# thu-ml/SageAttention

Hardware: AMD Instinct MI355X
Metric: attention TFLOPS (causal, hd=128), kernel-only, as published by the reference (higher is better)
Workload: dtype int8 QK^T + fp8(e4m3) PV, fp32 accumulate

## Files before the change

sageattention_amd/csrc/sage_prepass.hip:

```cpp
#include "sage_common.h"
#include "sage_kernels.h"
#include "sage_quant_math.h"
#include <type_traits>

#ifndef SAGE_PP_RELEASE
#define SAGE_PP_RELEASE 0
#endif
#ifndef SAGE_PP_NT
#define SAGE_PP_NT 1
#endif
#ifndef SAGE_PP_TRACE
#define SAGE_PP_TRACE 0
#endif
#ifndef SAGE_PP_KWB
#define SAGE_PP_KWB 1
#endif
#ifndef SAGE_PP_VAMAX
#define SAGE_PP_VAMAX 1
#endif
#ifndef SAGE_PP_ABL
#define SAGE_PP_ABL 0
#endif

namespace sage {

template <int DT> __device__ __forceinline__ void round_pair_to_dtype(float &a, float &b)
{
    if constexpr (DT == DT_BF16) {
        typedef float f2 __attribute__((ext_vector_type(2)));
        typedef __bf16 b2 __attribute__((ext_vector_type(2)));
        const b2 r = __builtin_convertvector(f2{a, b}, b2);
        unsigned u;
        __builtin_memcpy(&u, &r, 4);
        a = __uint_as_float(u << 16);
        b = __uint_as_float(u & 0xffff0000u);
    } else {
        a = f16_to_f32(f32_to_f16_rne(a));
        b = f16_to_f32(f32_to_f16_rne(b));
    }
}

constexpr int kPrepassThreads = 512;

template <int DT> __device__ __forceinline__ unsigned pack_pair_to_dtype(float a, float b)
{
    typedef float f2 __attribute__((ext_vector_type(2)));
    unsigned u;
    if constexpr (DT == DT_BF16) {
        typedef __bf16 b2 __attribute__((ext_vector_type(2)));
        const b2 r = __builtin_convertvector(f2{a, b}, b2);
        __builtin_memcpy(&u, &r, 4);
    } else {
        typedef _Float16 h2 __attribute__((ext_vector_type(2)));
        const h2 r = __builtin_convertvector(f2{a, b}, h2);
        __builtin_memcpy(&u, &r, 4);
    }
    return u;
}

template <int D>
struct PrepassLds {
    static constexpr int TPR = D / 4, RPI = kPrepassThreads / TPR, LDT = D + 8;
    float red[3][RPI][D];
    __attribute__((aligned(16))) uint16_t tile[2][BLKK * LDT];
    float ch_mean[D], ch_recp[D];
    uint16_t kmean[D];
    unsigned failed;
    unsigned gmax[8][8];
    float gsc[8][8], gy[8][8];
};

template <int D, int DT, bool IS_V, bool VARLEN, bool V_AMAX = false>
__device__ __forceinline__ void prepass_body(const PrepassParams &p, PrepassLds<D> &lds, const int b)
{

    constexpr int NT = kPrepassThreads;
    constexpr int TPR = D / 4;
    constexpr int RPI = NT / TPR;
    constexpr int NR = kStatsSlab / RPI;
    constexpr int LDT = D + 8;
    auto &red = lds.red; auto &tile = lds.tile; auto &ch_mean = lds.ch_mean; auto &ch_recp = lds.ch_recp;
    auto &kmean = lds.kmean; auto &gmax = lds.gmax; auto &gsc = lds.gsc; auto &gy = lds.gy;
    bool failed = false;
    constexpr int is_v = IS_V ? 1 : 0;

    const int tid = threadIdx.x;
    const int gslab = blockIdx.x, h = blockIdx.y;
    int slab = gslab, L = p.L, nslab = p.nslab;
    long tok0 = 0, tile0 = 0;
    bool gap = false;
    if constexpr (VARLEN) {
        typedef const __attribute__((address_space(4))) int *cint_p;
        nslab = ((cint_p)p.hdr)[4];
        if (gslab >= nslab) return;
        const int seg = ((cint_p)p.slab_seq)[gslab];
        slab = gslab - ((cint_p)p.slab_first)[seg];
        int t0, len;
        varlen_segment((cint_p)p.cu, p.nseq, p.L, seg, t0, len);
        tok0 = t0;
        L = len;
        gap = seg >= p.nseq;
        if (gap && (IS_V || p.k_mean == nullptr)) return;
        tile0 = gap ? 0 : ((cint_p)p.cu_tiles)[seg];
    }
    const long bh = (long)b * p.H + h;
    const long x_sl = is_v ? p.v_sl : p.k_sl;
    const uint16_t *x = (is_v ? reinterpret_cast<const uint16_t *>(p.v) + (long)b * p.v_sb + (long)h * p.v_sh
                              : reinterpret_cast<const uint16_t *>(p.k) + (long)b * p.k_sb + (long)h * p.k_sh) + tok0 * x_sl;
    const int c4 = (tid % TPR) * 4, r0 = tid / TPR;
    const int row0 = slab * kStatsSlab;
    const int end = min(L, row0 + kStatsSlab);
    const int my_rows = (end - row0 - r0 + RPI - 1) / RPI;
#if SAGE_PP_TRACE
    unsigned long long *trace = reinterpret_cast<unsigned long long *>(p.ws + 2L * p.B * p.H * p.nslab * 3 * D) +
                                8L * (blockIdx.x + gridDim.x * (blockIdx.y + (long)gridDim.y * blockIdx.z));
    int tslot = 0;
#define SAGE_STAMP() do { if (tid == 0) trace[tslot] = wall_clock64(); tslot++; } while (0)
    SAGE_STAMP();
#else
#define SAGE_STAMP() do { } while (0)
#endif

    unsigned rw[NR][2];
    {
        const unsigned head_bytes = (unsigned)(((long)(L - 1) * x_sl + D) * 2);
        const __amdgpu_buffer_rsrc_t rsrc = __builtin_amdgcn_make_buffer_rsrc(const_cast<uint16_t *>(x), 0, head_bytes, 0x00020000);
        const unsigned toff = (unsigned)((row0 + r0) * (int)x_sl + c4) * 2u;
        const unsigned step = (unsigned)(RPI * (int)x_sl) * 2u;
        unsigned voff = toff;
#pragma unroll
        for (int i = 0; i < NR; i++) {
            const v2u t = __builtin_amdgcn_raw_buffer_load_b64(rsrc, voff, 0, 0);
            rw[i][0] = t[0]; rw[i][1] = t[1];
            voff += step;
            asm volatile("" : "+v"(voff));
        }
    }
#if SAGE_PP_TRACE
    { unsigned acc = 0;
#pragma unroll
      for (int i = 0; i < NR; i++) acc += rw[i][0] ^ rw[i][1];
      if (acc == 0x12345u) p.ws[0] = 1.0f; }
    SAGE_STAMP();
#endif

    const bool need_stats = IS_V ? (p.v_fp16 == 0) : (p.k_mean != nullptr);
    if (need_stats) {
        float mx[4], mn[4], sm[4];
#pragma unroll
        for (int j = 0; j < 4; j++) { mx[j] = -INFINITY; mn[j] = INFINITY; sm[j] = 0.0f; }
        if constexpr (V_AMAX) {
            typedef unsigned short us2 __attribute__((ext_vector_type(2)));
            us2 am01 = {0, 0}, am23 = {0, 0};
#pragma unroll
            for (int i = 0; i < ((SAGE_PP_ABL & 4) ? 0 : NR); i++) {
                const unsigned m0 = rw[i][0] & 0x7fff7fffu, m1 = rw[i][1] & 0x7fff7fffu;
                us2 a, b;
                __builtin_memcpy(&a, &m0, 4);
                __builtin_memcpy(&b, &m1, 4);
                am01 = __builtin_elementwise_max(am01, a);
                am23 = __builtin_elementwise_max(am23, b);
                asm volatile("" : "+v"(am01), "+v"(am23) :: "memory");
            }
            mx[0] = ld16<DT>(am01[0]); mx[1] = ld16<DT>(am01[1]); mx[2] = ld16<DT>(am23[0]); mx[3] = ld16<DT>(am23[1]);
#pragma unroll
            for (int j = 0; j < 4; j++) mn[j] = 0.0f;
        } else if (!(SAGE_PP_ABL & 4)) {
#pragma unroll
            for (int i = 0; i < NR; i++) {
                float pen = 0.0f;
                if constexpr (IS_V) pen = __uint_as_float((unsigned)((my_rows - 1 - i) >> 31) & 0xff800000u);
#pragma unroll
                for (int c = 0; c < 2; c++) {
                    const unsigned w = rw[i][c];
                    const float lo = ld16<DT>((uint16_t)(w & 0xffffu)), hi = ld16<DT>((uint16_t)(w >> 16));
                    if constexpr (IS_V) {
                        mx[2 * c] = fmaxf(mx[2 * c], lo + pen);         mn[2 * c] = fminf(mn[2 * c], lo - pen);
                        mx[2 * c + 1] = fmaxf(mx[2 * c + 1], hi + pen); mn[2 * c + 1] = fminf(mn[2 * c + 1], hi - pen);
                    }
                    sm[2 * c] += lo;
                    sm[2 * c + 1] += hi;
                }
                asm volatile("" : "+v"(sm[0]), "+v"(sm[1]), "+v"(sm[2]), "+v"(sm[3]) :: "memory");
            }
        }
#pragma unroll
        for (int j = 0; j < 4; j++) { red[0][r0][c4 + j] = mx[j]; red[1][r0][c4 + j] = mn[j]; red[2][r0][c4 + j] = sm[j]; }
        __syncthreads();
        float *ws = p.ws + (((long)is_v * p.B * p.H + bh) * p.nslab) * 3 * D;
        if (tid < D) {
            float a = -INFINITY, c = INFINITY, s = 0.0f;
#pragma unroll
            for (int r = 0; r < RPI; r++) { a = fmaxf(a, red[0][r][tid]); c = fminf(c, red[1][r][tid]); s += red[2][r][tid]; }
            float *mine = ws + (long)gslab * 3 * D;
            if constexpr (IS_V) __hip_atomic_store(mine + tid, a, __ATOMIC_RELAXED, __HIP_MEMORY_SCOPE_AGENT);
            if constexpr (IS_V && !V_AMAX) __hip_atomic_store(mine + D + tid, c, __ATOMIC_RELAXED, __HIP_MEMORY_SCOPE_AGENT);
            if constexpr (!V_AMAX) __hip_atomic_store(mine + 2 * D + tid, s, __ATOMIC_RELAXED, __HIP_MEMORY_SCOPE_AGENT);
        }
        SAGE_STAMP();
        unsigned *cnt = p.sync + ((long)is_v * p.B * p.H + bh) * kPrepassSyncStride;
        if (nslab > 1 && !(SAGE_PP_ABL & 1)) {
            asm volatile("s_waitcnt vmcnt(0)" ::: "memory");
            __syncthreads();
            if (tid == 0) {
                __hip_atomic_fetch_add(cnt, 1u, SAGE_PP_RELEASE ? __ATOMIC_RELEASE : __ATOMIC_RELAXED, __HIP_MEMORY_SCOPE_AGENT);
                const unsigned want = (unsigned)nslab + (p.debug_fail ? 1u : 0u);
                const long long bound = p.debug_fail ? 20000LL : 3000000LL;
                const unsigned min_polls = p.debug_fail ? (1u << 8) : (1u << 14);
                const long long t0 = wall_clock64();
                unsigned gave_up = 0, polls = 0;
                while (__hip_atomic_load(cnt, __ATOMIC_RELAXED, __HIP_MEMORY_SCOPE_AGENT) < want) {
                    __builtin_amdgcn_s_sleep(2);
                    if (++polls > min_polls && wall_clock64() - t0 > bound) {
                        __hip_atomic_store(cnt + 2, 1u, __ATOMIC_RELAXED, __HIP_MEMORY_SCOPE_AGENT);
                        if (p.host_flag != nullptr) __hip_atomic_store(p.host_flag, 1u, __ATOMIC_RELAXED, __HIP_MEMORY_SCOPE_SYSTEM);
                        gave_up = 1;
                        break;
                    }
                }
                lds.failed = gave_up;
            }
            __syncthreads();
            failed = lds.failed != 0;
        }
        SAGE_STAMP();
        float a = -INFINITY, c = INFINITY, s = 0.0f;
        if (failed) {
            for (int i = 0; i < nslab; i++) {
                const uint16_t *xi = x;
                int Li = L, si = i;
                if constexpr (VARLEN) {
                    typedef const __attribute__((address_space(4))) int *cint_p;
                    const int seg = ((cint_p)p.slab_seq)[i];
                    si = i - ((cint_p)p.slab_first)[seg];
                    int t0;
                    varlen_segment((cint_p)p.cu, p.nseq, p.L, seg, t0, Li);
                    xi = x + ((long)t0 - tok0) * x_sl;
                }
                const int rbeg = si * kStatsSlab + r0, rend = min(Li, si * kStatsSlab + kStatsSlab);
                float fx[4], fn[4], fs[4];
#pragma unroll
                for (int j = 0; j < 4; j++) { fx[j] = V_AMAX ? 0.0f : -INFINITY; fn[j] = V_AMAX ? 0.0f : INFINITY; fs[j] = 0.0f; }
                const __amdgpu_buffer_rsrc_t rs_i = __builtin_amdgcn_make_buffer_rsrc(const_cast<uint16_t *>(xi), 0,
                                                                                      (unsigned)(((long)(Li - 1) * x_sl + D) * 2), 0x00020000);
                unsigned vo = (unsigned)(rbeg * (int)x_sl + c4) * 2u;
#pragma nounroll
                for (int r = rbeg; r < rend; r += RPI) {
                    const v2u t = __builtin_amdgcn_raw_buffer_load_b64(rs_i, vo, 0, 0);
                    vo += (unsigned)(RPI * (int)x_sl) * 2u;
#pragma unroll
                    for (int j = 0; j < 4; j++) {
                        const unsigned w = t[j >> 1];
                        const float f = ld16<DT>((uint16_t)((j & 1) ? (w >> 16) : (w & 0xffffu)));
                        if constexpr (V_AMAX) fx[j] = fmaxf(fx[j], fabsf(f));
                        else if constexpr (IS_V) { fx[j] = fmaxf(fx[j], f); fn[j] = fminf(fn[j], f); fs[j] += f; }
                        else fs[j] += f;
                    }
                }
                __syncthreads();
#pragma unroll
                for (int j = 0; j < 4; j++) {
                    if constexpr (IS_V) red[0][r0][c4 + j] = fx[j];
                    if constexpr (IS_V && !V_AMAX) red[1][r0][c4 + j] = fn[j];
                    if constexpr (!V_AMAX) red[2][r0][c4 + j] = fs[j];
                }
                __syncthreads();
                if (tid < D) {
                    float ai = -INFINITY, ci = INFINITY, s_i = 0.0f;
#pragma unroll
                    for (int r = 0; r < RPI; r++) {
                        if constexpr (IS_V) ai = fmaxf(ai, red[0][r][tid]);
                        if constexpr (IS_V && !V_AMAX) ci = fminf(ci, red[1][r][tid]);
                        if constexpr (!V_AMAX) s_i += red[2][r][tid];
                    }
                    if constexpr (IS_V) a = fmaxf(a, ai);
                    if constexpr (IS_V && !V_AMAX) c = fminf(c, ci);
                    if constexpr (!V_AMAX) s += s_i;
                }
            }
        } else if (tid < D) {
            constexpr int NB = (D == 128) ? 16 : 8;
            for (int i0 = 0; i0 < nslab; i0 += NB) {
                float va[NB], vc[NB], vs[NB];
#pragma unroll
                for (int u = 0; u < NB; u++) {
                    const float *wi = ws + (long)min(i0 + u, nslab - 1) * 3 * D;
                    if constexpr (IS_V) va[u] = __hip_atomic_load(wi + tid, __ATOMIC_RELAXED, __HIP_MEMORY_SCOPE_AGENT);
                    if constexpr (IS_V && !V_AMAX) vc[u] = __hip_atomic_load(wi + D + tid, __ATOMIC_RELAXED, __HIP_MEMORY_SCOPE_AGENT);
                    if constexpr (!V_AMAX) vs[u] = __hip_atomic_load(wi + 2 * D + tid, __ATOMIC_RELAXED, __HIP_MEMORY_SCOPE_AGENT);
                }
#pragma unroll
                for (int u = 0; u < NB; u++) {
                    if (i0 + u < nslab) {
                        if constexpr (IS_V) a = fmaxf(a, va[u]);
                        if constexpr (IS_V && !V_AMAX) c = fminf(c, vc[u]);
                        if constexpr (!V_AMAX) s += vs[u];
                    }
                }
            }
        }
        if (tid < D) {
            if constexpr (!IS_V) {
                const uint16_t m = st16<DT>(s / (float)(VARLEN ? p.L : L));
                kmean[tid] = m;
                if (gslab == 0) reinterpret_cast<uint16_t *>(p.k_mean)[bh * D + tid] = m;
            } else {
                const bool smooth = p.v_mean != nullptr;
                const float lpad = (float)((L + 15) / 16 * 16);
                const float mean = smooth ? s / lpad : 0.0f;
                if constexpr (V_AMAX) c = 0.0f;
                if ((L & 15) != 0) { a = fmaxf(a, 0.0f); c = fminf(c, 0.0f); }
                const float am = fmaxf(fabsf(a - mean), fabsf(c - mean));
                ch_mean[tid] = mean;
                ch_recp[tid] = am > 0.0f ? p.scale_max / am : 0.0f;
                if (gslab == 0) {
                    p.v_scale[bh * D + tid] = am / p.scale_max;
                    if (smooth) p.v_mean[bh * D + tid] = mean;
                }
            }
        }
        __syncthreads();
        SAGE_STAMP();
        if (nslab > 1 && tid == 0 && !(SAGE_PP_ABL & 1)) {
            const unsigned left = __hip_atomic_fetch_add(cnt + 1, 1u, __ATOMIC_RELAXED, __HIP_MEMORY_SCOPE_AGENT);
            if (left == (unsigned)nslab - 1) {
                __hip_atomic_store(cnt, 0u, __ATOMIC_RELAXED, __HIP_MEMORY_SCOPE_AGENT);
                __hip_atomic_store(cnt + 1, 0u, __ATOMIC_RELAXED, __HIP_MEMORY_SCOPE_AGENT);
            }
        }
    }
    if (gap) return;
    if (SAGE_PP_ABL & 2) {
        unsigned acc = 0;
#pragma unroll
        for (int i = 0; i < NR; i++) acc += rw[i][0] + rw[i][1];
        if (acc == 0x12345u) p.ws[0] = 1.0f;
        return;
    }

    if constexpr (!IS_V) {
        const int blk = p.k_blk;
        const int bsh = (blk == 128) ? 7 : 6;
        const int nb = kStatsSlab >> bsh;
        const int ngroups = (p.k_gran == GR_BLOCK) ? 1 : 4 * (blk / p.k_warp);
        const bool smooth = p.k_mean != nullptr;
        const unsigned init_bits = (p.k_style == QS_CUDA) ? __float_as_uint(1e-7f) : 0u;
        if (tid < 64) gmax[tid >> 3][tid & 7] = init_bits;
        float mean4[4] = {0.0f, 0.0f, 0.0f, 0.0f};
        unsigned m01 = 0u, m23 = 0u;
        if (smooth) {
            m01 = (unsigned)kmean[c4] | ((unsigned)kmean[c4 + 1] << 16);
            m23 = (unsigned)kmean[c4 + 2] | ((unsigned)kmean[c4 + 3] << 16);
#pragma unroll
            for (int j = 0; j < 4; j++) mean4[j] = ld16<DT>(kmean[c4 + j]);
        }
#pragma unroll
        for (int i = 0; i < NR; i++) {
            const unsigned gone = (unsigned)((my_rows - 1 - i) >> 31);
            rw[i][0] |= m01 & gone;
            rw[i][1] |= m23 & gone;
        }
#if SAGE_PP_KWB
        if (smooth && p.k_style != QS_CUDA) {
#pragma unroll
            for (int i = 0; i < NR; i++) {
#pragma unroll
                for (int c = 0; c < 2; c++) {
                    unsigned u = rw[i][c];
                    const float lo = ld16<DT>((uint16_t)(u & 0xffffu)) - mean4[2 * c];
                    const float hi = ld16<DT>((uint16_t)(u >> 16)) - mean4[2 * c + 1];
                    u = pack_pair_to_dtype<DT>(lo, hi);
                    asm volatile("" : "+v"(u));
                    rw[i][c] = u;
                }
                asm volatile("" ::: "memory");
            }
        }
#endif
        __syncthreads();
        const int g_thread = group_of_row(r0 & (blk - 1), p.k_gran, p.k_warp);
        const int nblk_total = (L + blk - 1) >> bsh;
        const __amdgpu_buffer_rsrc_t orsrc = __builtin_amdgcn_make_buffer_rsrc(
            p.k_out + (long)b * p.ko_sb + (long)h * p.ko_sh + tok0 * p.ko_sl, 0, (unsigned)((long)(L - 1) * p.ko_sl + D), 0x00020000);
        const unsigned ooff = (unsigned)((row0 + r0) * (int)p.ko_sl + c4), ostep = (unsigned)(RPI * (int)p.ko_sl);

        auto quantise = [&](auto style_tag, auto smooth_tag) {
            constexpr int STYLE = decltype(style_tag)::value;
            constexpr bool SMOOTH = decltype(smooth_tag)::value;
            auto row_values = [&](int i, float (&f)[4]) {
#pragma unroll
                for (int c = 0; c < 2; c++) {
                    unsigned w = rw[i][c];
                    asm volatile("" : "+v"(w));
                    float lo = ld16<DT>((uint16_t)(w & 0xffffu)), hi = ld16<DT>((uint16_t)(w >> 16));
                    if constexpr (SMOOTH) {
                        lo -= mean4[2 * c];
                        hi -= mean4[2 * c + 1];
                        if (STYLE != 0) round_pair_to_dtype<DT>(lo, hi);
                    }
                    f[2 * c] = lo;
                    f[2 * c + 1] = hi;
                }
            };
            const int rb_mask = (blk / RPI) - 1;
            float amax = 0.0f;
            typedef unsigned short us2 __attribute__((ext_vector_type(2)));
            us2 amax16 = {0, 0};
#pragma unroll
            for (int i = 0; i < NR; i++) {
                if constexpr (STYLE == 0) {
                    float f[4];
                    row_values(i, f);
                    amax = fmaxf(fmaxf(amax, fmaxf(fabsf(f[0]), fabsf(f[1]))), fmaxf(fabsf(f[2]), fabsf(f[3])));
                } else {
#pragma unroll
                    for (int c = 0; c < 2; c++) {
                        unsigned u = rw[i][c];
                        if constexpr (SMOOTH) {
                            asm volatile("" : "+v"(u));
                            const float lo = ld16<DT>((uint16_t)(u & 0xffffu)) - mean4[2 * c];
                            const float hi = ld16<DT>((uint16_t)(u >> 16)) - mean4[2 * c + 1];
                            u = pack_pair_to_dtype<DT>(lo, hi);
                        }
                        const unsigned mag = u & 0x7fff7fffu;
                        us2 m2;
                        __builtin_memcpy(&m2, &mag, 4);
                        amax16 = __builtin_elementwise_max(amax16, m2);
                    }
                }
                if ((i & 1) && ((i & rb_mask) == rb_mask)) {
                    float m = amax;
                    if constexpr (STYLE != 0) { m = ld16<DT>(amax16[0] > amax16[1] ? amax16[0] : amax16[1]); amax16 = us2{0, 0}; }
                    m = fmaxf(m, __uint_as_float(__builtin_amdgcn_update_dpp(0, __float_as_uint(m), 0xB1, 0xf, 0xf, true)));
                    m = fmaxf(m, __uint_as_float(__builtin_amdgcn_update_dpp(0, __float_as_uint(m), 0x4E, 0xf, 0xf, true)));
                    m = fmaxf(m, __uint_as_float(__builtin_amdgcn_update_dpp(0, __float_as_uint(m), 0x141, 0xf, 0xf, true)));
                    m = fmaxf(m, __uint_as_float(__builtin_amdgcn_update_dpp(0, __float_as_uint(m), 0x140, 0xf, 0xf, true)));
                    m = fmaxf(m, __shfl_xor(m, 16));
                    if ((tid & 31) == 0) atomicMax(&gmax[(i * RPI) >> bsh][g_thread], __float_as_uint(m));
                    amax = 0.0f;
                }
                asm volatile("" : "+v"(amax), "+v"(amax16) :: "memory");
            }
            __syncthreads();
            SAGE_STAMP();
            if (tid < nb * ngroups) {
                const int kb = tid / ngroups, g = tid % ngroups;
                const int gb = slab * nb + kb;
                const float am = __uint_as_float(gmax[kb][g]);
                const float sc = quant_scale(am, p.k_style);
                gsc[kb][g] = sc;
                gy[kb][g] = (STYLE == 0) ? 127.0f / am : quant_recip(sc);
                float *ksc_out = VARLEN ? p.k_scale + (tile0 + gb) * p.H + h
                                        : p.k_scale + (bh * nblk_total + gb) * ngroups + g;
                if (gb < nblk_total) *ksc_out = sc;
            }
            __syncthreads();
            unsigned orun = ooff;
#pragma unroll
            for (int i = 0; i < NR; i += 2) {
                const float sc = gsc[(i * RPI) >> bsh][g_thread], y = gy[(i * RPI) >> bsh][g_thread];
#pragma unroll
                for (int u = 0; u < 2; u++) {
                    float f[4];
                    row_values(i + u, f);
                    int q[4];
                    if constexpr (STYLE == 0) {
#pragma unroll
                        for (int j = 0; j < 4; j++) q[j] = quant_round_cuda(f[j], y);
                    } else if constexpr (STYLE == 1) quant_round_triton_nz4(f, sc, y, q);
                    else quant_round_triton4(f, sc, y, q);
                    __builtin_amdgcn_raw_buffer_store_b32(pack_int8x4(q[0], q[1], q[2], q[3]), orsrc, orun, 0, SAGE_PP_NT ? 2 : 0);
                    orun += ostep;
                    asm volatile("" : "+v"(orun) :: "memory");
                }
            }
        };
        auto by_smooth = [&](auto style_tag) {
            if (smooth) quantise(style_tag, std::true_type{}); else quantise(style_tag, std::false_type{});
        };
        if (p.k_style == QS_CUDA) by_smooth(std::integral_constant<int, 0>{});
#if SAGE_PP_KWB
        else if (p.k_style == QS_TRITON_THREAD) quantise(std::integral_constant<int, 1>{}, std::false_type{});
        else quantise(std::integral_constant<int, 2>{}, std::false_type{});
#else
        else if (p.k_style == QS_TRITON_THREAD) by_smooth(std::integral_constant<int, 1>{});
        else by_smooth(std::integral_constant<int, 2>{});
#endif
    } else {
        const bool smooth = V_AMAX ? false : (p.v_mean != nullptr);
        const int ntiles = (L + BLKK - 1) / BLKK;
        constexpr int RPS = 2 * BLKK / RPI;
        auto stage_in = [&](int s) {
#pragma unroll
            for (int m = 0; m < RPS; m++) {
                const int rs = r0 + m * RPI;
                const v2u t = {rw[s * RPS + m][0], rw[s * RPS + m][1]};
                *reinterpret_cast<v2u *>(&tile[rs >> 6][(rs & 63) * LDT + c4]) = t;
            }
        };
        if (p.v_fp16 == 0) {
            unsigned char *img = reinterpret_cast<unsigned char *>(p.v_image) + bh * (long)ntiles * (D * 64);
#pragma unroll
            for (int s = 0; s < kStatsSlab / (2 * BLKK); s++) {
                if (row0 + s * 2 * BLKK < L) {
                    stage_in(s);
                    __syncthreads();
#pragma unroll
                    for (int it = 0; it < 2 * D * 4 / NT; it++) {
                        const int piece = tid + NT * it;
                        const int tt = piece / (D * 4), pin = piece % (D * 4);
                        const int d = pin >> 2, pc = pin & 3;
                        const int t = (row0 >> 6) + 2 * s + tt;
                        if (t >= ntiles) continue;
                        const int ch = swz_chunk<64>(d, pc);
                        const float mean = ch_mean[d], recp = ch_recp[d];
                        float f[16];
#pragma unroll
                        for (int j = 0; j < 16; j++) {
                            const int tok = pv_token_of_position(16 * ch + j);
                            float xv = ld16<DT>(tile[tt][tok * LDT + d]);
                            if (smooth) xv = (t * BLKK + tok < L) ? xv - mean : 0.0f;
                            xv *= recp;
                            f[j] = fminf(fmaxf(xv, -448.0f), 448.0f);
                        }
                        v4u pk;
#pragma unroll
                        for (int w = 0; w < 4; w++) {
                            int word = __builtin_amdgcn_cvt_pk_fp8_f32(f[4 * w], f[4 * w + 1], 0, false);
                            word = __builtin_amdgcn_cvt_pk_fp8_f32(f[4 * w + 2], f[4 * w + 3], word, true);
                            pk[w] = (unsigned)word;
                        }
                        if constexpr (SAGE_PP_NT != 0) __builtin_nontemporal_store(pk, reinterpret_cast<v4u *>(img + (long)t * (D * 64) + d * 64 + pc * 16));
                        else *reinterpret_cast<v4u *>(img + (long)t * (D * 64) + d * 64 + pc * 16) = pk;
                    }
                    __syncthreads();
                }
            }
        } else {
            const long img_t = VARLEN ? (long)p.H * (D * 128) : (long)(D * 128);
            unsigned char *img = reinterpret_cast<unsigned char *>(p.v_image) + (VARLEN ? (tile0 * p.H + h) * (long)(D * 128) : bh * (long)ntiles * (D * 128));
#pragma unroll
            for (int s = 0; s < kStatsSlab / (2 * BLKK); s++) {
                if (row0 + s * 2 * BLKK < L) {
                    stage_in(s);
                    __syncthreads();
#pragma unroll
                    for (int it = 0; it < 2 * D * 8 / NT; it++) {
                        const int piece = tid + NT * it;
                        const int tt = piece / (D * 8), pin = piece % (D * 8);
                        const int d = pin >> 3, pc = pin & 7;
                        const int t = (row0 >> 6) + 2 * s + tt;
                        if (t >= ntiles) continue;
                        const int ch = swz_chunk<128>(d, pc);
                        v4u pk;
#pragma unroll
                        for (int w = 0; w < 4; w++) {
                            unsigned word = 0;
#pragma unroll
                            for (int e = 0; e < 2; e++) {
                                const int tok = pv_token_of_position(8 * ch + 2 * w + e);
                                uint16_t raw = tile[tt][tok * LDT + d];
                                if (DT != DT_F16) raw = f32_to_f16_rne(bf16_to_f32(raw));
                                word |= (unsigned)raw << (16 * e);
                            }
                            pk[w] = word;
                        }
                        if constexpr (SAGE_PP_NT != 0) __builtin_nontemporal_store(pk, reinterpret_cast<v4u *>(img + (long)t * img_t + d * 128 + pc * 16));
                        else *reinterpret_cast<v4u *>(img + (long)t * img_t + d * 128 + pc * 16) = pk;
                    }
                    __syncthreads();
                }
            }
        }
    }
#if SAGE_PP_TRACE
    asm volatile("s_waitcnt vmcnt(0)" ::: "memory");
    if (is_v) tslot = 6;
    SAGE_STAMP();
    if (tid == 0) trace[7] = (unsigned long long)__builtin_amdgcn_s_getreg((3 << 11) | 20) |
                              ((unsigned long long)__builtin_amdgcn_s_getreg((31 << 11) | 4) << 8);
#endif
}

template <int D, int DT, bool VARLEN>
#ifndef SAGE_PP_WAVES
#define SAGE_PP_WAVES 4
#endif
#ifndef SAGE_PP_WAVES64
#define SAGE_PP_WAVES64 6
#endif
__global__ void __launch_bounds__(kPrepassThreads, (D == 64 ? SAGE_PP_WAVES64 : SAGE_PP_WAVES))
prepass_kv_kernel(const PrepassParams p)
{
    __shared__ PrepassLds<D> lds;
    const int is_v = (p.parts == 3) ? (int)(blockIdx.z & 1) : (p.parts == 2);
    const int b = (p.parts == 3) ? (int)(blockIdx.z >> 1) : (int)blockIdx.z;
    if (is_v) {
        if (SAGE_PP_VAMAX && !VARLEN && p.v_mean == nullptr && p.v_fp16 == 0) prepass_body<D, DT, true, VARLEN, true>(p, lds, b);
        else prepass_body<D, DT, true, VARLEN>(p, lds, b);
    } else prepass_body<D, DT, false, VARLEN>(p, lds, b);
}

__global__ void __launch_bounds__(1024) debug_spin_kernel(long long ticks)
{
    const long long t0 = wall_clock64();
    while (wall_clock64() - t0 < ticks) __builtin_amdgcn_s_sleep(8);
}

hipError_t launch_debug_spin(int ms, int nwg, hipStream_t s)
{
    hipLaunchKernelGGL(debug_spin_kernel, dim3(nwg), dim3(1024), 0, s, (long long)ms * 100000LL);
    return hipGetLastError();
}

hipError_t launch_prepass_kv(const PrepassParams &p, hipStream_t s)
{
    if (p.B <= 0 || p.H <= 0 || p.nslab <= 0 || p.parts == 0) return hipSuccess;
    dim3 grid(p.nslab, p.H, p.B * (p.parts == 3 ? 2 : 1));
#define SAGE_PP(D_, T_) do { if (p.cu != nullptr) hipLaunchKernelGGL((prepass_kv_kernel<D_, T_, true>), grid, dim3(kPrepassThreads), 0, s, p); \
                             else hipLaunchKernelGGL((prepass_kv_kernel<D_, T_, false>), grid, dim3(kPrepassThreads), 0, s, p); } while (0)
    if (p.D == 128) { if (p.dtype == DT_F16) SAGE_PP(128, DT_F16); else SAGE_PP(128, DT_BF16); }
    else if (p.D == 64) { if (p.dtype == DT_F16) SAGE_PP(64, DT_F16); else SAGE_PP(64, DT_BF16); }
    else return hipErrorInvalidValue;
#undef SAGE_PP
    return hipGetLastError();
}

}
```

Before: 1612.

## Use swizzled LDS units with transpose reads and double-buffering in V prepass

Replaces the padded LDS tile in the V prepass with XOR-swizzled unit buffers (one aliased with the reduction scratch) that are read back through ds_read_tr16 transpose loads. Each lane now gathers four tokens per instruction instead of scalar 16-bit loads. Staging of the next unit is overlapped with converting the current one, which removes one barrier per step. It also drops unused stats reductions, skips the K padding fix-up when the slab is full, moves the gmax init earlier to remove a barrier, and swaps a shuffle for permlane16_swap. In exchange the swizzle and lane-mapping logic is intricate and relies on gfx950-only instructions.

```diff
diff --git a/sageattention_amd/csrc/sage_prepass.hip b/sageattention_amd/csrc/sage_prepass.hip
--- a/sageattention_amd/csrc/sage_prepass.hip
+++ b/sageattention_amd/csrc/sage_prepass.hip
@@ -60,9 +60,18 @@
 
 template <int D>
 struct PrepassLds {
-    static constexpr int TPR = D / 4, RPI = kPrepassThreads / TPR, LDT = D + 8;
-    float red[3][RPI][D];
-    __attribute__((aligned(16))) uint16_t tile[2][BLKK * LDT];
+    static constexpr int TPR = D / 4, RPI = kPrepassThreads / TPR;
+    static constexpr int UT = BLKK * 8 / (D / 16), UNIT = UT * D;
+    union {
+        __attribute__((aligned(16))) float red[3][RPI][D];
+        __attribute__((aligned(16))) uint16_t unit1[UNIT];
+    };
+    __attribute__((aligned(16))) uint16_t unit0[UNIT];
+    static __device__ __forceinline__ int tile_off(int row, int chunk, int col)
+    {
+        const int swz = (D == 128) ? ((row & 7) ^ ((row >> 2) & 4)) : (((row >> 1) & 3) ^ ((row >> 3) & 2));
+        return row * D + 16 * (chunk ^ swz) + col;
+    }
     float ch_mean[D], ch_recp[D];
     uint16_t kmean[D];
     unsigned failed;
@@ -78,8 +87,7 @@
     constexpr int TPR = D / 4;
     constexpr int RPI = NT / TPR;
     constexpr int NR = kStatsSlab / RPI;
-    constexpr int LDT = D + 8;
-    auto &red = lds.red; auto &tile = lds.tile; auto &ch_mean = lds.ch_mean; auto &ch_recp = lds.ch_recp;
+    auto &red = lds.red; auto &ch_mean = lds.ch_mean; auto &ch_recp = lds.ch_recp;
     auto &kmean = lds.kmean; auto &gmax = lds.gmax; auto &gsc = lds.gsc; auto &gy = lds.gy;
     bool failed = false;
     constexpr int is_v = IS_V ? 1 : 0;
@@ -145,6 +153,10 @@
 #endif
 
     const bool need_stats = IS_V ? (p.v_fp16 == 0) : (p.k_mean != nullptr);
+    if constexpr (!IS_V) {
+        const unsigned init_bits = (p.k_style == QS_CUDA) ? __float_as_uint(1e-7f) : 0u;
+        if (tid < 64) gmax[tid >> 3][tid & 7] = init_bits;
+    }
     if (need_stats) {
         float mx[4], mn[4], sm[4];
 #pragma unroll
@@ -185,13 +197,21 @@
             }
         }
 #pragma unroll
-        for (int j = 0; j < 4; j++) { red[0][r0][c4 + j] = mx[j]; red[1][r0][c4 + j] = mn[j]; red[2][r0][c4 + j] = sm[j]; }
+        for (int j = 0; j < 4; j++) {
+            if constexpr (IS_V) red[0][r0][c4 + j] = mx[j];
+            if constexpr (IS_V && !V_AMAX) red[1][r0][c4 + j] = mn[j];
+            if constexpr (!V_AMAX) red[2][r0][c4 + j] = sm[j];
+        }
         __syncthreads();
         float *ws = p.ws + (((long)is_v * p.B * p.H + bh) * p.nslab) * 3 * D;
         if (tid < D) {
             float a = -INFINITY, c = INFINITY, s = 0.0f;
 #pragma unroll
-            for (int r = 0; r < RPI; r++) { a = fmaxf(a, red[0][r][tid]); c = fminf(c, red[1][r][tid]); s += red[2][r][tid]; }
+            for (int r = 0; r < RPI; r++) {
+                if constexpr (IS_V) a = fmaxf(a, red[0][r][tid]);
+                if constexpr (IS_V && !V_AMAX) c = fminf(c, red[1][r][tid]);
+                if constexpr (!V_AMAX) s += red[2][r][tid];
+            }
             float *mine = ws + (long)gslab * 3 * D;
             if constexpr (IS_V) __hip_atomic_store(mine + tid, a, __ATOMIC_RELAXED, __HIP_MEMORY_SCOPE_AGENT);
             if constexpr (IS_V && !V_AMAX) __hip_atomic_store(mine + D + tid, c, __ATOMIC_RELAXED, __HIP_MEMORY_SCOPE_AGENT);
@@ -344,8 +364,6 @@
         const int nb = kStatsSlab >> bsh;
         const int ngroups = (p.k_gran == GR_BLOCK) ? 1 : 4 * (blk / p.k_warp);
         const bool smooth = p.k_mean != nullptr;
-        const unsigned init_bits = (p.k_style == QS_CUDA) ? __float_as_uint(1e-7f) : 0u;
-        if (tid < 64) gmax[tid >> 3][tid & 7] = init_bits;
         float mean4[4] = {0.0f, 0.0f, 0.0f, 0.0f};
         unsigned m01 = 0u, m23 = 0u;
         if (smooth) {
@@ -354,11 +372,13 @@
 #pragma unroll
             for (int j = 0; j < 4; j++) mean4[j] = ld16<DT>(kmean[c4 + j]);
         }
-#pragma unroll
-        for (int i = 0; i < NR; i++) {
-            const unsigned gone = (unsigned)((my_rows - 1 - i) >> 31);
-            rw[i][0] |= m01 & gone;
-            rw[i][1] |= m23 & gone;
+        if (smooth && end - row0 < kStatsSlab) {
+#pragma unroll
+            for (int i = 0; i < NR; i++) {
+                const unsigned gone = (unsigned)((my_rows - 1 - i) >> 31);
+                rw[i][0] |= m01 & gone;
+                rw[i][1] |= m23 & gone;
+            }
         }
 #if SAGE_PP_KWB
         if (smooth && p.k_style != QS_CUDA) {
@@ -377,7 +397,7 @@
             }
         }
 #endif
-        __syncthreads();
+        if (!need_stats) __syncthreads();
         const int g_thread = group_of_row(r0 & (blk - 1), p.k_gran, p.k_warp);
         const int nblk_total = (L + blk - 1) >> bsh;
         const __amdgpu_buffer_rsrc_t orsrc = __builtin_amdgcn_make_buffer_rsrc(
@@ -435,7 +455,10 @@
                     m = fmaxf(m, __uint_as_float(__builtin_amdgcn_update_dpp(0, __float_as_uint(m), 0x4E, 0xf, 0xf, true)));
                     m = fmaxf(m, __uint_as_float(__builtin_amdgcn_update_dpp(0, __float_as_uint(m), 0x141, 0xf, 0xf, true)));
                     m = fmaxf(m, __uint_as_float(__builtin_amdgcn_update_dpp(0, __float_as_uint(m), 0x140, 0xf, 0xf, true)));
-                    m = fmaxf(m, __shfl_xor(m, 16));
+                    {
+                        const auto sw = __builtin_amdgcn_permlane16_swap(__float_as_uint(m), __float_as_uint(m), false, false);
+                        m = fmaxf(__uint_as_float(sw[0]), __uint_as_float(sw[1]));
+                    }
                     if ((tid & 31) == 0) atomicMax(&gmax[(i * RPI) >> bsh][g_thread], __float_as_uint(m));
                     amax = 0.0f;
                 }
@@ -489,88 +512,105 @@
     } else {
         const bool smooth = V_AMAX ? false : (p.v_mean != nullptr);
         const int ntiles = (L + BLKK - 1) / BLKK;
-        constexpr int RPS = 2 * BLKK / RPI;
-        auto stage_in = [&](int s) {
-#pragma unroll
-            for (int m = 0; m < RPS; m++) {
-                const int rs = r0 + m * RPI;
-                const v2u t = {rw[s * RPS + m][0], rw[s * RPS + m][1]};
-                *reinterpret_cast<v2u *>(&tile[rs >> 6][(rs & 63) * LDT + c4]) = t;
+        typedef short v4s __attribute__((ext_vector_type(4)));
+        typedef __attribute__((address_space(3))) v4s *lds_v4s;
+        constexpr int NCG = D / 16;
+        constexpr int UT = PrepassLds<D>::UT;
+        constexpr int RPU = UT / RPI;
+        const int wave = tid >> 6, l16 = tid & 15, grp = (tid >> 4) & 3;
+        const int tt = wave / NCG, cg = wave % NCG;
+        auto unit_in = [&](int u) {
+            uint16_t *dst = (u & 1) ? lds.unit1 : lds.unit0;
+#pragma unroll
+            for (int m = 0; m < RPU; m++) {
+                const v2u t = {rw[u * RPU + m][0], rw[u * RPU + m][1]};
+                *reinterpret_cast<v2u *>(&dst[PrepassLds<D>::tile_off(r0 + m * RPI, c4 >> 4, c4 & 15)]) = t;
+            }
+        };
+        auto tokens4 = [&](int u, int tok) {
+            const uint16_t *src = (u & 1) ? lds.unit1 : lds.unit0;
+            return __builtin_amdgcn_ds_read_tr16_b64_v4i16((lds_v4s)&src[PrepassLds<D>::tile_off(64 * tt + tok + (l16 >> 2), cg, 4 * (l16 & 3))]);
+        };
+        auto run_units = [&](auto convert) {
+            unit_in(0);
+            __syncthreads();
+#pragma unroll
+            for (int u = 0; u < kStatsSlab / UT; u++) {
+                if (row0 + u * UT < L) {
+                    const bool more = u + 1 < kStatsSlab / UT && row0 + (u + 1) * UT < L;
+                    if (more) unit_in(u + 1);
+                    const int t = (row0 >> 6) + u * (UT / BLKK) + tt;
+                    if (t < ntiles) convert(u, t);
+                    if (more) __syncthreads();
+                }
             }
         };
         if (p.v_fp16 == 0) {
             unsigned char *img = reinterpret_cast<unsigned char *>(p.v_image) + bh * (long)ntiles * (D * 64);
-#pragma unroll
-            for (int s = 0; s < kStatsSlab / (2 * BLKK); s++) {
-                if (row0 + s * 2 * BLKK < L) {
-                    stage_in(s);
-                    __syncthreads();
-#pragma unroll
-                    for (int it = 0; it < 2 * D * 4 / NT; it++) {
-                        const int piece = tid + NT * it;
-                        const int tt = piece / (D * 4), pin = piece % (D * 4);
-                        const int d = pin >> 2, pc = pin & 3;
-                        const int t = (row0 >> 6) + 2 * s + tt;
-                        if (t >= ntiles) continue;
-                        const int ch = swz_chunk<64>(d, pc);
-                        const float mean = ch_mean[d], recp = ch_recp[d];
-                        float f[16];
-#pragma unroll
-                        for (int j = 0; j < 16; j++) {
-                            const int tok = pv_token_of_position(16 * ch + j);
-                            float xv = ld16<DT>(tile[tt][tok * LDT + d]);
-                            if (smooth) xv = (t * BLKK + tok < L) ? xv - mean : 0.0f;
-                            xv *= recp;
-                            f[j] = fminf(fmaxf(xv, -448.0f), 448.0f);
-                        }
-                        v4u pk;
-#pragma unroll
-                        for (int w = 0; w < 4; w++) {
-                            int word = __builtin_amdgcn_cvt_pk_fp8_f32(f[4 * w], f[4 * w + 1], 0, false);
-                            word = __builtin_amdgcn_cvt_pk_fp8_f32(f[4 * w + 2], f[4 * w + 3], word, true);
-                            pk[w] = (unsigned)word;
-                        }
-                        if constexpr (SAGE_PP_NT != 0) __builtin_nontemporal_store(pk, reinterpret_cast<v4u *>(img + (long)t * (D * 64) + d * 64 + pc * 16));
-                        else *reinterpret_cast<v4u *>(img + (long)t * (D * 64) + d * 64 + pc * 16) = pk;
-                    }
-                    __syncthreads();
-                }
-            }
+            const int ch = ((grp & 1) << 1) | (grp >> 1);
+            const int d = 16 * cg + l16, pc = ch ^ ((d >> 2) & 3);
+            run_units([&](int u, int t) {
+                const float mean = ch_mean[d], recp = ch_recp[d];
+                float f[16];
+#pragma unroll
+                for (int w = 0; w < 4; w++) {
+                    const int tok0w = pv_token_of_position(16 * ch + 4 * w);
+                    const v4s r = tokens4(u, tok0w);
+#pragma unroll
+                    for (int q = 0; q < 4; q++) {
+                        float xv = ld16<DT>((uint16_t)r[q]);
+                        if (smooth) xv = (t * BLKK + tok0w + q < L) ? xv - mean : 0.0f;
+                        xv *= recp;
+                        f[4 * w + q] = fminf(fmaxf(xv, -448.0f), 448.0f);
+                    }
+                }
+                v4u pk;
+#pragma unroll
+                for (int w = 0; w < 4; w++) {
+                    int word = __builtin_amdgcn_cvt_pk_fp8_f32(f[4 * w], f[4 * w + 1], 0, false);
+                    word = __builtin_amdgcn_cvt_pk_fp8_f32(f[4 * w + 2], f[4 * w + 3], word, true);
+                    pk[w] = (unsigned)word;
+                }
+                if constexpr (SAGE_PP_NT != 0) __builtin_nontemporal_store(pk, reinterpret_cast<v4u *>(img + (long)t * (D * 64) + d * 64 + pc * 16));
+                else *reinterpret_cast<v4u *>(img + (long)t * (D * 64) + d * 64 + pc * 16) = pk;
+            });
         } else {
             const long img_t = VARLEN ? (long)p.H * (D * 128) : (long)(D * 128);
             unsigned char *img = reinterpret_cast<unsigned char *>(p.v_image) + (VARLEN ? (tile0 * p.H + h) * (long)(D * 128) : bh * (long)ntiles * (D * 128));
-#pragma unroll
-            for (int s = 0; s < kStatsSlab / (2 * BLKK); s++) {
-                if (row0 + s * 2 * BLKK < L) {
-                    stage_in(s);
-                    __syncthreads();
-#pragma unroll
-                    for (int it = 0; it < 2 * D * 8 / NT; it++) {
-                        const int piece = tid + NT * it;
-                        const int tt = piece / (D * 8), pin = piece % (D * 8);
-                        const int d = pin >> 3, pc = pin & 7;
-                        const int t = (row0 >> 6) + 2 * s + tt;
-                        if (t >= ntiles) continue;
-                        const int ch = swz_chunk<128>(d, pc);
-                        v4u pk;
-#pragma unroll
-                        for (int w = 0; w < 4; w++) {
-                            unsigned word = 0;
-#pragma unroll
-                            for (int e = 0; e < 2; e++) {
-                                const int tok = pv_token_of_position(8 * ch + 2 * w + e);
-                                uint16_t raw = tile[tt][tok * LDT + d];
-                                if (DT != DT_F16) raw = f32_to_f16_rne(bf16_to_f32(raw));
-                                word |= (unsigned)raw << (16 * e);
-                            }
-                            pk[w] = word;
+            const bool lo8 = l16 < 8;
+            run_units([&](int u, int t) {
+                v4u pa, pb;
+#pragma unroll
+                for (int rd = 0; rd < 2; rd++) {
+                    const int tok0r = pv_token_of_position(8 * grp + 4 * rd);
+                    const v4s ra = tokens4(u, tok0r), rb = tokens4(u, tok0r + 4);
+#pragma unroll
+                    for (int e = 0; e < 2; e++) {
+                        uint16_t a0 = (uint16_t)ra[2 * e], a1 = (uint16_t)ra[2 * e + 1], b0 = (uint16_t)rb[2 * e], b1 = (uint16_t)rb[2 * e + 1];
+                        if (DT != DT_F16) {
+                            a0 = f32_to_f16_rne(bf16_to_f32(a0)); a1 = f32_to_f16_rne(bf16_to_f32(a1));
+                            b0 = f32_to_f16_rne(bf16_to_f32(b0)); b1 = f32_to_f16_rne(bf16_to_f32(b1));
                         }
-                        if constexpr (SAGE_PP_NT != 0) __builtin_nontemporal_store(pk, reinterpret_cast<v4u *>(img + (long)t * img_t + d * 128 + pc * 16));
-                        else *reinterpret_cast<v4u *>(img + (long)t * img_t + d * 128 + pc * 16) = pk;
-                    }
-                    __syncthreads();
-                }
-            }
+                        pa[2 * rd + e] = (unsigned)a0 | ((unsigned)a1 << 16);
+                        pb[2 * rd + e] = (unsigned)b0 | ((unsigned)b1 << 16);
+                    }
+                }
+                v4u s0, s1;
+#pragma unroll
+                for (int k = 0; k < 4; k++) {
+                    const unsigned got = __builtin_amdgcn_update_dpp(0, lo8 ? pb[k] : pa[k], 0x128, 0xf, 0xf, true);
+                    s0[k] = lo8 ? pa[k] : got;
+                    s1[k] = lo8 ? got : pb[k];
+                }
+                const int chs = grp + 4 * (l16 >> 3);
+#pragma unroll
+                for (int hf = 0; hf < 2; hf++) {
+                    const int d = 16 * cg + 8 * hf + (l16 & 7), pc = chs ^ ((d >> 1) & 7);
+                    const v4u pk = hf ? s1 : s0;
+                    if constexpr (SAGE_PP_NT != 0) __builtin_nontemporal_store(pk, reinterpret_cast<v4u *>(img + (long)t * img_t + d * 128 + pc * 16));
+                    else *reinterpret_cast<v4u *>(img + (long)t * img_t + d * 128 + pc * 16) = pk;
+                }
+            });
         }
     }
 #if SAGE_PP_TRACE
```

Result: no change. 1611 (-0.1%).
